# joeyan/gaussian_splatting

Hardware: AMD Instinct MI355X
Metric: forward+backward Mpixels/s @ ~1MP, N Gaussians; grad max-rel-err vs ref (higher is better)
Workload: dtype f32; 1 GPU; D: 2860000 Gaussians, 1297x840, SH degree 3, seed 0; N=2860000, V=2751015, P=1089480, camera=fixed, parallelism=single

## Files before the change

### gaussian_splatting_amd/csrc/gs_common.h

```cpp
#pragma once
#include <hip/hip_runtime.h>
#include <stdint.h>

#include "../../include/gsplat_hip.h"

#define GS_WAVE 64

namespace gs {

void set_error(const char* fmt, ...);
int check_launch(const char* what);

#define GS_REQUIRE(cond, ...)                                                                      \
    do {                                                                                           \
        if (!(cond)) {                                                                             \
            gs::set_error(__VA_ARGS__);                                                            \
            return GS_EINVAL;                                                                      \
        }                                                                                          \
    } while (0)

__host__ __device__ inline float bits_f(uint32_t u) {
    union { uint32_t u; float f; } c;
    c.u = u;
    return c.f;
// ... 24 lines not shown
    p = __builtin_fmaf(p, f, 1.33335581464284e-3f);
    p = __builtin_fmaf(p, f, 9.61812910762848e-3f);
    p = __builtin_fmaf(p, f, 5.55041086648216e-2f);
    p = __builtin_fmaf(p, f, 2.40226506959101e-1f);
    p = __builtin_fmaf(p, f, 6.93147180559945e-1f);
    p = __builtin_fmaf(p, f, 1.0f);
    float r = __builtin_ldexpf(p, (int)n);
    r = (t > 127.0f) ? __builtin_inff() : r;
    r = (t > -125.0f) ? r : 0.0f;
    r = (t != t) ? t : r;
    return r;
}

template <typename T> __device__ inline T gexp(T x);
template <> __device__ inline float gexp<float>(float x) { return det_expf(x); }
template <> __device__ inline double gexp<double>(double x) { return exp(x); }

template <typename T> __device__ inline T gsqrt(T x);
template <> __device__ inline float gsqrt<float>(float x) { return __builtin_sqrtf(x); }
template <> __device__ inline double gsqrt<double>(double x) { return __builtin_sqrt(x); }

__device__ inline int f2i(float x) {
    if (x != x) return 0;
    if (x >= 2147483648.0f) return 2147483647;
    if (x <= -2147483648.0f) return (-2147483647 - 1);
    return (int)x;
}

template <typename T, int RA, int CA, int CB>
__device__ inline void matmul(const T* A, const T* B, T* C) {
#pragma unroll
    for (int r = 0; r < RA; r++)
#pragma unroll
        for (int c = 0; c < CB; c++) {
            T sum = 0;
#pragma unroll
            for (int k = 0; k < CA; k++) sum += A[r * CA + k] * B[k * CB + c];
            C[r * CB + c] = sum;
        }
}
template <typename T, int R, int C>
__device__ inline void transp(const T* A, T* At) {
#pragma unroll
    for (int r = 0; r < R; r++)
#pragma unroll
        for (int c = 0; c < C; c++) At[c * R + r] = A[r * C + c];
}

#define GS_SH_0 0.28209479177387814f
#define GS_R_SH_0 3.544907701811032f
#define GS_SH_1 0.4886025119029199f
#define GS_SH_2_0 1.0925484305920792f
#define GS_SH_2_2 0.31539156525252005f
#define GS_SH_2_4 0.5462742152960396f
#define GS_SH_3_0 0.5900435899266435f
#define GS_SH_3_1 2.890611442640554f
#define GS_SH_3_2 0.4570457994644658f
#define GS_SH_3_3 0.263875515352797f
#define GS_SH_3_5 1.445305721320277f

template <typename T, int N_SH>
__device__ inline void sh_basis(const T* d, T* Y) {
    Y[0] = T(GS_SH_0);
    if constexpr (N_SH >= 4) {
        const T x = d[0], y = d[1], z = d[2];
        Y[1] = T(-GS_SH_1) * y;
        Y[2] = T(GS_SH_1) * z;
        Y[3] = T(-GS_SH_1) * x;
        if constexpr (N_SH >= 9) {
            const T xy = x * y, yz = y * z, xz = x * z, xx = x * x, yy = y * y, zz = z * z;
            Y[4] = T(GS_SH_2_0) * xy;
            Y[5] = T(-GS_SH_2_0) * yz;
            Y[6] = T(GS_SH_2_2) * (3 * zz - 1.0);
            Y[7] = T(-GS_SH_2_0) * xz;
            Y[8] = T(GS_SH_2_4) * (xx - yy);
            if constexpr (N_SH >= 16) {
                Y[9] = T(-GS_SH_3_0) * y * (3 * xx - yy);
                Y[10] = T(GS_SH_3_1) * xy * z;
                Y[11] = T(-GS_SH_3_2) * y * (5 * zz - 1.0);
                Y[12] = T(GS_SH_3_3) * z * (5 * zz - 3.0);
                Y[13] = T(-GS_SH_3_2) * x * (5 * zz - 1.0);
                Y[14] = T(GS_SH_3_5) * z * (xx - yy);
                Y[15] = T(-GS_SH_3_0) * x * (xx - 3 * yy);
            }
        }
    }
}

template <typename T, int N_SH>
__device__ inline void sh_to_rgb(const T* coeff, const T* Y, T* rgb) {
#pragma unroll
    for (int c = 0; c < 3; c++) rgb[c] = Y[0] * coeff[N_SH * c];
    if constexpr (N_SH >= 4) {
#pragma unroll
        for (int s = 1; s < N_SH; s++)
#pragma unroll
            for (int c = 0; c < 3; c++) rgb[c] += Y[s] * coeff[N_SH * c + s];
    }
}

template <typename T, int N_SH>
__device__ inline void sh_to_rgb_contracted(const T* coeff, const T* Y, T* rgb) {
#pragma clang fp contract(fast)
#pragma unroll
    for (int c = 0; c < 3; c++) rgb[c] = Y[0] * coeff[N_SH * c];
    if constexpr (N_SH >= 4) {
#pragma unroll
        for (int s = 1; s < N_SH; s++)
#pragma unroll
            for (int c = 0; c < 3; c++) rgb[c] += Y[s] * coeff[N_SH * c + s];
    }
}

constexpr int SORT_MAX_LDS_KEYS = 8192;
__host__ __device__ inline bool prefix_sorted_tile(int n, int sort_prefix) {
    return sort_prefix > 0 && n > sort_prefix && n <= SORT_MAX_LDS_KEYS;
}

int sort_flagged_tiles(const int* ranges, const uint64_t* keys, int* sorted, int tile0, int nt,
                       int64_t S, const int* flags, hipStream_t s);

constexpr int DC_PART = 256;
struct CutState {
    int* ctrl;
    int* totals;
    int* bstar;
    int* boff;
    int* boff2;
    uint32_t* bounds;
    int* phist;
    int* list;
    uint16_t* bucket_of;
};
__host__ __device__ inline size_t cut_ws_ints(int N, int T) {
    const size_t n = (size_t)(N > 0 ? N : 1), t = (size_t)(T > 0 ? T : 1);
    return 8 + 2 * t + 2 * (GS_CUT_BUCKETS + 8) + GS_CUT_BUCKETS + (size_t)DC_PART * GS_CUT_BUCKETS + n + (n + 1) / 2 + 16;
}
__host__ __device__ inline CutState cut_state_of(int32_t* ws, int N, int T) {
    const size_t n = (size_t)(N > 0 ? N : 1), t = (size_t)(T > 0 ? T : 1);
    CutState c;
    int* p = ws;
    c.ctrl = p; p += 8;
    c.totals = p; p += t;
    c.bstar = p; p += t;
    c.boff = p; p += GS_CUT_BUCKETS + 8;
    c.boff2 = p; p += GS_CUT_BUCKETS + 8;
    c.bounds = (uint32_t*)p; p += GS_CUT_BUCKETS;
    c.phist = p; p += (size_t)DC_PART * GS_CUT_BUCKETS;
    c.list = p; p += n;
    c.bucket_of = (uint16_t*)p;
    return c;
}

int depth_cut_repair(const float* bin_records, int N, int ntx, int nty, float mh, int row0, int row1,
                     const int* full_ranges, int32_t* workspace, int32_t* cut_ws, uint64_t* okeys, int64_t ocap,
                     int* osorted, const int* flags, hipStream_t s, bool sort_too = true);
int* depth_cut_flag_counter(int32_t* cut_ws, int N, int T);

inline int div_up(int a, int b) { return (a + b - 1) / b; }

}
```

### gaussian_splatting_amd/csrc/gs_error.hip

```cpp
#include <stdarg.h>
#include <stdio.h>

#include "gs_common.h"

namespace gs {

static thread_local char g_err[512] = "";

void set_error(const char* fmt, ...) {
    va_list ap;
    va_start(ap, fmt);
    vsnprintf(g_err, sizeof(g_err), fmt, ap);
    va_end(ap);
}

int check_launch(const char* what) {
    hipError_t e = hipGetLastError();
    if (e != hipSuccess) {
        set_error("%s: %s", what, hipGetErrorString(e));
        return GS_EHIP;
    }
    return GS_OK;
}

}

extern "C" {
const char* gs_last_error(void) { return gs::g_err; }
int gs_abi_version(void) { return 15; }
}
```

### gaussian_splatting_amd/csrc/preprocess.hip

```cpp
#include <type_traits>

#include "adam_math.h"
#include "pg_math.h"
#include "tile_math.h"

namespace gs {

constexpr int PP_BLOCK = 256;

struct Frustum {
    float near, far, u_lo, u_hi, v_lo, v_hi;
};

__device__ inline void camera_center(const float* __restrict__ M, float* __restrict__ center) {
    const double a = M[0], b = M[1], c = M[2], d = M[4], e = M[5], f = M[6], g = M[8], h = M[9],
                 i = M[10];
    const double tx = M[3], ty = M[7], tz = M[11];
    const double A = e * i - f * h, B = -(d * i - f * g), C = d * h - e * g;
    const double det = a * A + b * B + c * C;
    const double inv[9] = {A / det, -(b * i - c * h) / det, (b * f - c * e) / det,
                           B / det, (a * i - c * g) / det, -(a * f - c * d) / det,
                           C / det, -(a * h - b * g) / det, (a * e - b * d) / det};
    center[0] = (float)(-(inv[0] * tx + inv[1] * ty + inv[2] * tz));
    center[1] = (float)(-(inv[3] * tx + inv[4] * ty + inv[5] * tz));
    center[2] = (float)(-(inv[6] * tx + inv[7] * ty + inv[8] * tz));
}

__device__ inline void to_camera(const float* __restrict__ M, float x, float y, float z, float* c) {
    c[0] = M[0] * x + M[1] * y + M[2] * z + M[3];
    c[1] = M[4] * x + M[5] * y + M[6] * z + M[7];
    c[2] = M[8] * x + M[9] * y + M[10] * z + M[11];
}

__device__ inline bool is_culled(const float* c, const float* __restrict__ K, const Frustum& fr,
                                 float* uv) {
    uv[0] = K[0] * c[0] / c[2] + K[2];
    uv[1] = K[4] * c[1] / c[2] + K[5];
    return (c[2] < fr.near) | (c[2] > fr.far) | (uv[0] < fr.u_lo) | (uv[0] > fr.u_hi) |
           (uv[1] < fr.v_lo) | (uv[1] > fr.v_hi);
}

__device__ inline int depth_bin(float z, const Frustum& fr) {
    const uint32_t lo = sortable_bits(fr.near), hi = sortable_bits(fr.far);
    const uint64_t range = (uint64_t)(hi - lo) + 1;
    const uint32_t x = min(max(sortable_bits(z), lo), hi);
    return (int)(((uint64_t)(x - lo) * GS_CUT_HIST_BINS) / range);
}

__global__ __launch_bounds__(PP_BLOCK) void k_cull_count(const float* __restrict__ xyz,
                                                         const float* __restrict__ M,
                                                         const float* __restrict__ K, int N,
                                                         Frustum fr, int* __restrict__ block_counts,
                                                         float* __restrict__ center,
                                                         int* __restrict__ depth_hist, int sample_stride) {
    __shared__ int s_cnt[PP_BLOCK / GS_WAVE];
    const int g = blockIdx.x * PP_BLOCK + threadIdx.x;
    if (g == 0) camera_center(M, center);
    bool vis = false;
    if (g < N) {
        float c[3], uv[2];
        to_camera(M, xyz[g * 3 + 0], xyz[g * 3 + 1], xyz[g * 3 + 2], c);
        vis = !is_culled(c, K, fr, uv);
        if (depth_hist != nullptr && vis && g % sample_stride == 0)
            atomicAdd(&depth_hist[depth_bin(c[2], fr)], 1);
    }
    const int n = __popcll(__ballot(vis));
    if ((threadIdx.x & 63) == 0) s_cnt[threadIdx.x >> 6] = n;
    __syncthreads();
    if (threadIdx.x == 0) block_counts[blockIdx.x] = s_cnt[0] + s_cnt[1] + s_cnt[2] + s_cnt[3];
}

template <bool CUT>
__global__ __launch_bounds__(1024) void k_scan_counts(const int* __restrict__ counts, int n,
                                                      int* __restrict__ offsets,
                                                      int* __restrict__ total_out, int* __restrict__ depth_hist,
                                                      uint32_t* __restrict__ bounds, Frustum fr) {
    __shared__ int s_wave[16];
    __shared__ int s_carry;
    __shared__ int s_cum[CUT ? GS_CUT_HIST_BINS : 1];
    const int tid = threadIdx.x, lane = tid & 63, wave = tid >> 6;
    if constexpr (CUT) if (blockIdx.x == 1) {
        constexpr int PER = GS_CUT_HIST_BINS / 1024;
        static_assert(GS_CUT_HIST_BINS % 1024 == 0 && GS_CUT_BUCKETS == 1024, "one thread per bucket, PER bins per thread");
        int v[PER], sum = 0;
#pragma unroll
        for (int k = 0; k < PER; k++) {
            v[k] = depth_hist[tid * PER + k];
            depth_hist[tid * PER + k] = 0;
            sum += v[k];
        }
        int incl = sum;
#pragma unroll
        for (int d = 1; d < 64; d <<= 1) {
            const int o = __shfl_up(incl, d);
            if (lane >= d) incl += o;
        }
        if (lane == 63) s_wave[wave] = incl;
        __syncthreads();
        int run = incl - sum, valid = 0;
        for (int w = 0; w < 16; w++) {
            if (w < wave) run += s_wave[w];
            valid += s_wave[w];
        }
#pragma unroll
        for (int k = 0; k < PER; k++) {
            run += v[k];
            s_cum[tid * PER + k] = run;
        }
        __syncthreads();
        uint32_t bound = 0xffffffffu;
        if (tid < GS_CUT_BUCKETS - 1 && valid > 0) {
            const int64_t target_num = (int64_t)(tid + 1) * valid;
            int lo_i = 0, len = GS_CUT_HIST_BINS;
            while (len > 0) {
                const int half = len >> 1;
                if ((int64_t)s_cum[lo_i + half] * GS_CUT_BUCKETS < target_num) {
                    lo_i += half + 1;
                    len -= half + 1;
                } else {
                    len = half;
                }
            }
            const int j = min(lo_i, GS_CUT_HIST_BINS - 1);
            const int64_t prev = j > 0 ? s_cum[j - 1] : 0, h = max(s_cum[j] - (int)prev, 1);
            const uint32_t lo = sortable_bits(fr.near), hi = sortable_bits(fr.far);
            const uint64_t range = (uint64_t)(hi - lo) + 1;
            const double frac = (double)(target_num - prev * GS_CUT_BUCKETS) / ((double)h * GS_CUT_BUCKETS);
            const double pos = ((double)j + frac) / (double)GS_CUT_HIST_BINS;
            const uint64_t b = (uint64_t)lo + (uint64_t)(pos * (double)range);
            bound = (uint32_t)min(b, (uint64_t)hi);
        }
        if (tid < GS_CUT_BUCKETS) bounds[tid] = bound;
        return;
    }
    if (tid == 0) s_carry = 0;
    __syncthreads();
    for (int base = 0; base < n; base += 4096) {
        int v[4], sum = 0;
#pragma unroll
        for (int k = 0; k < 4; k++) {
            const int i = base + tid * 4 + k;
            v[k] = i < n ? counts[i] : 0;
            sum += v[k];
        }
        int incl = sum;
#pragma unroll
        for (int d = 1; d < 64; d <<= 1) {
            const int o = __shfl_up(incl, d);
            if (lane >= d) incl += o;
        }
        if (lane == 63) s_wave[wave] = incl;
        __syncthreads();
        int off = s_carry;
        for (int w = 0; w < wave; w++) off += s_wave[w];
        int run = off + incl - sum;
#pragma unroll
        for (int k = 0; k < 4; k++) {
            const int i = base + tid * 4 + k;
            if (i < n) offsets[i] = run;
            run += v[k];
        }
        __syncthreads();
        if (tid == 1023) s_carry = run;
        __syncthreads();
    }
    if (tid == 0) total_out[0] = s_carry;
}

__device__ inline float sigmoid_det(float x) { return 1.0f / (1.0f + det_expf(-x)); }

struct PreOut {
    float* uv;
    float* conic;
    float* opacity;
    float* rgb;
    float* xyz_cam;
    float* packed;
    int* vis_idx;
    int* rank;
    uint8_t* culled;
    float* bin_rec;
    const uint32_t* bounds;
    uint16_t* bucket_of;
};

struct Band {
    int row0, row1, ntx, nty;
    float mh;
};

template <int N_SH, bool BAND, bool AA = false>
__global__ __launch_bounds__(PP_BLOCK) __attribute__((amdgpu_waves_per_eu(5, 8))) void k_preprocess(
    const float* __restrict__ xyz, const float* __restrict__ quat, const float* __restrict__ scale,
    const float* __restrict__ opacity, const float* __restrict__ rgb, const float* __restrict__ sh,
    const float* __restrict__ M, const float* __restrict__ K, const float* __restrict__ center,
    int N, Frustum fr, const int* __restrict__ block_offsets, PreOut o, Band band) {
    __shared__ int s_cnt[PP_BLOCK / GS_WAVE];
    constexpr int SHW = 3 * (N_SH - 1);
    constexpr int HALF = PP_BLOCK / 2;
    __shared__ alignas(16) float s_sh[(N_SH > 1 && !BAND) ? HALF * SHW : 4];
    __shared__ uint32_t s_bounds[BAND ? 1 : GS_CUT_BUCKETS];
    const int g = blockIdx.x * PP_BLOCK + threadIdx.x;
    const int lane = threadIdx.x & 63, wave = threadIdx.x >> 6;
    if constexpr (!BAND) {
        if (o.bin_rec != nullptr)
            for (int k = threadIdx.x; k < GS_CUT_BUCKETS; k += PP_BLOCK) s_bounds[k] = o.bounds[k];
    }
    bool vis = false;
    float c[3] = {0, 0, 1}, uv[2] = {0, 0}, p[3] = {0, 0, 0};
    typedef float vfloat4 __attribute__((ext_vector_type(4)));
    constexpr int SH_PRE = (N_SH > 1 && !BAND) ? (HALF * SHW / 4 + PP_BLOCK - 1) / PP_BLOCK : 1;
    vfloat4 pre[2][SH_PRE];
    float q4[4] = {0, 0, 0, 1}, s3[3] = {0, 0, 0}, opa_raw = 0;
    if (g < N) {
        p[0] = xyz[g * 3 + 0]; p[1] = xyz[g * 3 + 1]; p[2] = xyz[g * 3 + 2];
        if constexpr (!BAND) {
            q4[0] = quat[g * 4 + 0]; q4[1] = quat[g * 4 + 1]; q4[2] = quat[g * 4 + 2]; q4[3] = quat[g * 4 + 3];
            s3[0] = scale[g * 3 + 0]; s3[1] = scale[g * 3 + 1]; s3[2] = scale[g * 3 + 2];
            opa_raw = opacity[g];
        }
    }
    if constexpr (N_SH > 1 && !BAND) {
// ... 754 lines not shown
#pragma unroll
        for (int k = 0; k < 3; k++) {
            adam_update(as_p[k], gs[k], as_m[k], as_v[k], S.w1, S.beta2, S.w2, ad.scale.bc2_sqrt, S.eps, ad.scale.neg_step);
            ad.scale.p[g * 3 + k] = as_p[k]; ad.scale.m[g * 3 + k] = as_m[k]; ad.scale.v[g * 3 + k] = as_v[k];
            adam_update(ac_p[k], gc[k], ac_m[k], ac_v[k], S.w1, S.beta2, S.w2, ad.rgb.bc2_sqrt, S.eps, ad.rgb.neg_step);
            ad.rgb.p[g * 3 + k] = ac_p[k]; ad.rgb.m[g * 3 + k] = ac_m[k]; ad.rgb.v[g * 3 + k] = ac_v[k];
        }
        adam_update(ao_p, go, ao_m, ao_v, S.w1, S.beta2, S.w2, ad.opacity.bc2_sqrt, S.eps, ad.opacity.neg_step);
        ad.opacity.p[g] = ao_p; ad.opacity.m[g] = ao_m; ad.opacity.v[g] = ao_v;
        return;
    }
    o.quaternion[g * 4 + 0] = gq[0]; o.quaternion[g * 4 + 1] = gq[1];
    o.quaternion[g * 4 + 2] = gq[2]; o.quaternion[g * 4 + 3] = gq[3];
    o.scale[g * 3 + 0] = gs[0]; o.scale[g * 3 + 1] = gs[1]; o.scale[g * 3 + 2] = gs[2];
    o.opacity[g] = go;
    o.rgb[g * 3 + 0] = gc[0]; o.rgb[g * 3 + 1] = gc[1]; o.rgb[g * 3 + 2] = gc[2];
}

constexpr int POSE_MAX_BLOCKS = 2048;
constexpr int POSE_SUM_BLOCK = 1024;

inline int pose_blocks(int N) {
    const int nb = N > 0 ? div_up(N, PP_BLOCK) : 0;
    return nb < POSE_MAX_BLOCKS ? nb : POSE_MAX_BLOCKS;
}

struct NoOpacity {};
template <bool AA = false>
__global__ __launch_bounds__(PP_BLOCK) void k_pose_bwd(
    const float* __restrict__ xyz, const float* __restrict__ quat, const float* __restrict__ scale,
    const float* __restrict__ M, const float* __restrict__ K, const int* __restrict__ rank,
    const float* __restrict__ g_slab, int v_base, int N, float* __restrict__ rows,
    std::conditional_t<AA, const float*, NoOpacity> opacity_act = {}) {
    __shared__ float s_part[PP_BLOCK / GS_WAVE][12];
    float acc[12];
#pragma unroll
    for (int k = 0; k < 12; k++) acc[k] = 0.0f;
    float W[9];
    load_rotation(M, W);
    const float fx = K[0], fy = K[4];
    for (int g = blockIdx.x * PP_BLOCK + threadIdx.x; g < N; g += gridDim.x * PP_BLOCK) {
        const int v = rank[g];
        if (v < 0) continue;
        const float* gsl = g_slab + (size_t)(v - v_base) * 9;
        const float p[3] = {xyz[g * 3 + 0], xyz[g * 3 + 1], xyz[g * 3 + 2]};
        const float q4[4] = {quat[g * 4 + 0], quat[g * 4 + 1], quat[g * 4 + 2], quat[g * 4 + 3]};
        const float s3[3] = {scale[g * 3 + 0], scale[g * 3 + 1], scale[g * 3 + 2]};
        float c[3], S9[9], J6[6], gJ6[6], gW9[9], gcam[3];
        to_camera(M, p[0], p[1], p[2], c);
        sigma_world_of(q4, s3, S9);
        const float z = c[2], z2 = c[2] * c[2];
        J6[0] = fx / z; J6[1] = 0; J6[2] = -fx * c[0] / z2;
        J6[3] = 0; J6[4] = fy / z; J6[5] = -fy * c[1] / z2;
        float gc3[3] = {gsl[6], gsl[7], gsl[8]};
        if constexpr (AA) {
            float c3[3], g_opa = gsl[3];
            conic_of(J6, W, S9, c3);
            aa_fold_row(aa_terms_of(c3), opacity_act[v], g_opa, gc3);
        }
        conic_bwd_pose_of(J6, W, S9, gc3, gJ6, gW9);
        cam_grad_of(c, fx, fy, gJ6, gsl + 4, gcam);
#pragma unroll
        for (int i = 0; i < 3; i++) {
#pragma unroll
            for (int j = 0; j < 3; j++) acc[4 * i + j] += gW9[3 * i + j] + gcam[i] * p[j];
            acc[4 * i + 3] += gcam[i];
        }
    }
#pragma unroll
    for (int k = 0; k < 12; k++)
#pragma unroll
        for (int d = 1; d < GS_WAVE; d <<= 1) acc[k] += __shfl_xor(acc[k], d);
    if ((threadIdx.x & (GS_WAVE - 1)) == 0)
#pragma unroll
        for (int k = 0; k < 12; k++) s_part[threadIdx.x / GS_WAVE][k] = acc[k];
    __syncthreads();
    static_assert(PP_BLOCK / GS_WAVE == 4, "the workgroup sum below names its four waves");
    if (threadIdx.x < 12)
        rows[blockIdx.x * 12 + threadIdx.x] = (s_part[0][threadIdx.x] + s_part[1][threadIdx.x]) +
                                              (s_part[2][threadIdx.x] + s_part[3][threadIdx.x]);
}

__global__ __launch_bounds__(POSE_SUM_BLOCK) void k_pose_sum(const float* __restrict__ rows, int n_rows,
                                                             float* __restrict__ out) {
    __shared__ double s_sum[POSE_SUM_BLOCK / 16][12];
    const int k = threadIdx.x & 15, r0 = threadIdx.x >> 4;
    if (k < 12) {
        double sum = 0.0;
        for (int r = r0; r < n_rows; r += POSE_SUM_BLOCK / 16) sum += (double)rows[(size_t)r * 12 + k];
        s_sum[r0][k] = sum;
    }
    __syncthreads();
    if (threadIdx.x < 12) {
        double sum = 0.0;
        for (int r = 0; r < POSE_SUM_BLOCK / 16; r++) sum += s_sum[r][threadIdx.x];
        out[threadIdx.x] = (float)sum;
    } else if (threadIdx.x < 16) {
        out[threadIdx.x] = 0.0f;
    }
}

}

using namespace gs;

static Frustum make_frustum(int W, int H, float near, float far, float padding) {
    Frustum fr;
    fr.near = near;
    fr.far = far;
    fr.u_lo = -1.0f * padding;
    fr.u_hi = (float)W + padding;
    fr.v_lo = -1.0f * padding;
    fr.v_hi = (float)H + padding;
    return fr;
}

#define DISPATCH_SH(n_sh, CALL)                                                                    \
    switch (n_sh) {                                                                                \
        case 1: { constexpr int N_SH = 1; CALL; } break;                                           \
        case 4: { constexpr int N_SH = 4; CALL; } break;                                           \
        case 9: { constexpr int N_SH = 9; CALL; } break;                                           \
        case 16: { constexpr int N_SH = 16; CALL; } break;                                         \
        default:                                                                                   \
            gs::set_error("Unsupported number of SH coefficients: %d", n_sh);                      \
            return GS_EINVAL;                                                                      \
    }

#define GS_RASTER_MODE(raster_mode, aa)                                                                      \
    GS_REQUIRE((raster_mode) == GS_RASTER_CLASSIC || (raster_mode) == GS_RASTER_ANTIALIASED,               \
               "raster_mode must be GS_RASTER_CLASSIC or GS_RASTER_ANTIALIASED, got %d", (int)(raster_mode)); \
    const bool aa = (raster_mode) == GS_RASTER_ANTIALIASED

static int preprocess_forward_launch(const void* xyz, const void* quaternion, const void* scale,
                                     const void* opacity, const void* rgb, const void* sh, int n_sh,
                                     const void* camera_T_world, const void* K, int N, int W, int H,
                                     float near_thresh, float far_thresh, float cull_mask_padding,
                                     float mh_dist, int band_row0, int band_row1,
                                     int32_t* workspace, void* camera_center, int32_t* visible_count,
                                     uint8_t* culling_mask, int32_t* rank, int32_t* vis_idx, void* uv,
                                     void* xyz_camera_frame, void* conic, void* opacity_act, void* rgb_render,
                                     void* packed, void* bin_records, int32_t* cut_workspace, int32_t* depth_hist,
                                     int sample_stride, bool aa, void* stream) {
    GS_REQUIRE((bin_records == nullptr) == (cut_workspace == nullptr) && (bin_records == nullptr) == (depth_hist == nullptr),
               "bin_records, cut_workspace and depth_hist go together");
    GS_REQUIRE(depth_hist == nullptr || sample_stride >= 1, "sample_stride must be gs_cut_sample_stride(N)");
    GS_REQUIRE(bin_records != nullptr || (uv != nullptr && xyz_camera_frame != nullptr && conic != nullptr),
               "uv, xyz_camera_frame and conic may only be omitted together with bin_records");
    GS_REQUIRE(n_sh == 1 || sh != nullptr, "sh must be given when n_sh > 1");
    hipStream_t s = (hipStream_t)stream;
    const Frustum fr = make_frustum(W, H, near_thresh, far_thresh, cull_mask_padding);
    const int nb = div_up(N > 0 ? N : 1, PP_BLOCK);
    int* block_counts = workspace;
    int* block_offsets = workspace + nb;
    k_cull_count<<<nb, PP_BLOCK, 0, s>>>((const float*)xyz, (const float*)camera_T_world,
                                         (const float*)K, N, fr, block_counts, (float*)camera_center, depth_hist,
                                         sample_stride > 0 ? sample_stride : 1);
    const int n_tiles = ((W + GS_TILE - 1) / GS_TILE) * ((H + GS_TILE - 1) / GS_TILE);
    CutState cs{};
    if (cut_workspace != nullptr) {
        cs = cut_state_of(cut_workspace, N, n_tiles);
        k_scan_counts<true><<<2, 1024, 0, s>>>(block_counts, nb, block_offsets, visible_count, depth_hist, cs.bounds, fr);
    } else {
        k_scan_counts<false><<<1, 1024, 0, s>>>(block_counts, nb, block_offsets, visible_count, nullptr, nullptr, fr);
    }
    PreOut o;
    o.uv = (float*)uv;
    o.conic = (float*)conic;
    o.opacity = (float*)opacity_act;
    o.rgb = (float*)rgb_render;
    o.xyz_cam = (float*)xyz_camera_frame;
    o.packed = (float*)packed;
    o.vis_idx = vis_idx;
    o.rank = rank;
    o.culled = culling_mask;
    o.bin_rec = (float*)bin_records;
    o.bounds = cs.bounds;
    o.bucket_of = cs.bucket_of;
    Band band;
    band.ntx = (W + GS_TILE - 1) / GS_TILE;
    band.nty = (H + GS_TILE - 1) / GS_TILE;
    band.row0 = band_row0;
    band.row1 = band_row1;
    band.mh = mh_dist;
    GS_REQUIRE(band_row0 >= 0 && band_row1 <= band.nty && band_row0 <= band_row1, "bad tile row band");
    const bool banded = !(band_row0 == 0 && band_row1 == band.nty);
    GS_REQUIRE(!(banded && bin_records != nullptr), "the depth-bucketed binning serves whole frames");
    GS_REQUIRE(!(banded && aa), "GS_RASTER_ANTIALIASED serves whole frames (no tile-row band)");
    if (aa) {
        DISPATCH_SH(n_sh, (k_preprocess<N_SH, false, true><<<nb, PP_BLOCK, 0, s>>>(
                              (const float*)xyz, (const float*)quaternion, (const float*)scale,
                              (const float*)opacity, (const float*)rgb, (const float*)sh,
                              (const float*)camera_T_world, (const float*)K,
                              (const float*)camera_center, N, fr, block_offsets, o, band)));
    } else if (banded) {
        DISPATCH_SH(n_sh, (k_preprocess<N_SH, true><<<nb, PP_BLOCK, 0, s>>>(
                              (const float*)xyz, (const float*)quaternion, (const float*)scale,
                              (const float*)opacity, (const float*)rgb, (const float*)sh,
                              (const float*)camera_T_world, (const float*)K,
                              (const float*)camera_center, N, fr, block_offsets, o, band)));
    } else {
        DISPATCH_SH(n_sh, (k_preprocess<N_SH, false><<<nb, PP_BLOCK, 0, s>>>(
                              (const float*)xyz, (const float*)quaternion, (const float*)scale,
                              (const float*)opacity, (const float*)rgb, (const float*)sh,
                              (const float*)camera_T_world, (const float*)K,
                              (const float*)camera_center, N, fr, block_offsets, o, band)));
    }
    return check_launch("preprocess_forward");
}

extern "C" {

size_t gs_preprocess_workspace_ints(int N) { return (size_t)div_up(N > 0 ? N : 1, PP_BLOCK) * 2 + 8; }

int gs_preprocess_forward_cut(const void* xyz, const void* quaternion, const void* scale,
                              const void* opacity, const void* rgb, const void* sh, int n_sh,
                              const void* camera_T_world, const void* K, int N, int W, int H,
                              float near_thresh, float far_thresh, float cull_mask_padding,
                              float mh_dist, int band_row0, int band_row1,
                              int32_t* workspace, void* camera_center, int32_t* visible_count,
                              uint8_t* culling_mask, int32_t* rank, int32_t* vis_idx, void* uv,
                              void* xyz_camera_frame, void* conic, void* opacity_act, void* rgb_render,
                              void* packed, void* bin_records, int32_t* cut_workspace, int32_t* depth_hist,
                              int sample_stride, void* stream) {
    return preprocess_forward_launch(xyz, quaternion, scale, opacity, rgb, sh, n_sh, camera_T_world, K, N, W, H, near_thresh,
                                     far_thresh, cull_mask_padding, mh_dist, band_row0, band_row1, workspace, camera_center,
                                     visible_count, culling_mask, rank, vis_idx, uv, xyz_camera_frame, conic, opacity_act,
                                     rgb_render, packed, bin_records, cut_workspace, depth_hist, sample_stride, false, stream);
}

int gs_preprocess_forward_mode(const void* xyz, const void* quaternion, const void* scale,
                               const void* opacity, const void* rgb, const void* sh, int n_sh,
                               const void* camera_T_world, const void* K, int N, int W, int H,
                               float near_thresh, float far_thresh, float cull_mask_padding,
                               float mh_dist, int band_row0, int band_row1,
                               int32_t* workspace, void* camera_center, int32_t* visible_count,
                               uint8_t* culling_mask, int32_t* rank, int32_t* vis_idx, void* uv,
                               void* xyz_camera_frame, void* conic, void* opacity_act, void* rgb_render,
                               void* packed, void* bin_records, int32_t* cut_workspace, int32_t* depth_hist,
                               int sample_stride, int raster_mode, void* stream) {
    GS_RASTER_MODE(raster_mode, aa);
    return preprocess_forward_launch(xyz, quaternion, scale, opacity, rgb, sh, n_sh, camera_T_world, K, N, W, H, near_thresh,
                                     far_thresh, cull_mask_padding, mh_dist, band_row0, band_row1, workspace, camera_center,
                                     visible_count, culling_mask, rank, vis_idx, uv, xyz_camera_frame, conic, opacity_act,
                                     rgb_render, packed, bin_records, cut_workspace, depth_hist, sample_stride, aa, stream);
}


int gs_band_project(const void* xyz, const void* scale, const void* opacity, const void* camera_T_world, const void* K,
                    int N, int W, int H, float near_thresh, float far_thresh, float cull_mask_padding, float mh_dist,
                    const int32_t* band_rows, int G, int32_t* workspace, void* camera_center, int32_t* visible_count,
                    uint8_t* culling_mask, int32_t* rank, int32_t* vis_idx, void* uv, void* opacity_act, uint32_t* mask,
                    int32_t* halo_workspace, void* stream) {
    GS_REQUIRE(G >= 1 && G <= GS_MAX_RANKS, "band_project: 1 <= G <= %d", GS_MAX_RANKS);
    hipStream_t s = (hipStream_t)stream;
    const Frustum fr = make_frustum(W, H, near_thresh, far_thresh, cull_mask_padding);
    const int nb = div_up(N > 0 ? N : 1, PP_BLOCK);
    int* block_counts = workspace;
    int* block_offsets = workspace + nb;
    k_cull_count<<<nb, PP_BLOCK, 0, s>>>((const float*)xyz, (const float*)camera_T_world, (const float*)K, N, fr,
                                         block_counts, (float*)camera_center, nullptr, 1);
    k_scan_counts<false><<<1, 1024, 0, s>>>(block_counts, nb, block_offsets, visible_count, nullptr, nullptr, fr);
    BandRows rows;
    for (int i = 0; i <= GS_MAX_RANKS; i++) rows.v[i] = i <= G ? band_rows[i] : 0;
    const int nty = (H + GS_TILE - 1) / GS_TILE;
    k_band_project<1><<<nb, PP_BLOCK, 0, s>>>((const float*)xyz, (const float*)scale, (const float*)opacity,
                                              (const float*)camera_T_world, (const float*)K, N, fr, mh_dist, nty, rows, G,
                                              block_offsets, culling_mask, rank, vis_idx, (float*)uv, (float*)opacity_act,
                                              mask, nullptr, nb);
    k_band_bit_counts<<<nb, PP_BLOCK, 0, s>>>(mask, visible_count, G, halo_workspace, nb);
    return check_launch("band_project");
}

int gs_preprocess_forward(const void* xyz, const void* quaternion, const void* scale,
                          const void* opacity, const void* rgb, const void* sh, int n_sh,
                          const void* camera_T_world, const void* K, int N, int W, int H,
                          float near_thresh, float far_thresh, float cull_mask_padding,
                          float mh_dist, int band_row0, int band_row1,
                          int32_t* workspace, void* camera_center, int32_t* visible_count,
                          uint8_t* culling_mask, int32_t* rank, int32_t* vis_idx, void* uv,
                          void* xyz_camera_frame, void* conic, void* opacity_act, void* rgb_render,
                          void* packed, void* stream) {
    return gs_preprocess_forward_cut(xyz, quaternion, scale, opacity, rgb, sh, n_sh, camera_T_world, K, N, W, H, near_thresh,
                                     far_thresh, cull_mask_padding, mh_dist, band_row0, band_row1, workspace, camera_center,
                                     visible_count, culling_mask, rank, vis_idx, uv, xyz_camera_frame, conic, opacity_act,
                                     rgb_render, packed, nullptr, nullptr, nullptr, 0, stream);
}

int gs_preprocess_forward_list(const void* xyz, const void* quaternion, const void* scale, const void* rgb, const void* sh,
                               int n_sh, const void* camera_T_world, const void* K, const void* camera_center,
                               const int32_t* list, const int32_t* list_count, int capacity, const int32_t* vis_idx,
                               const void* uv, const void* opacity_act, void* uv_l, void* xyz_camera_frame_l, void* conic_l,
                               void* packed_l, void* stream) {
    GS_REQUIRE(n_sh == 1 || sh != nullptr, "sh must be given when n_sh > 1");
    if (capacity <= 0) return GS_OK;
    hipStream_t s = (hipStream_t)stream;
    DISPATCH_SH(n_sh, (k_preprocess_list<N_SH><<<div_up(capacity, PP_BLOCK), PP_BLOCK, 0, s>>>(
                          (const float*)xyz, (const float*)quaternion, (const float*)scale, (const float*)rgb,
                          (const float*)sh, (const float*)camera_T_world, (const float*)K, (const float*)camera_center, list,
                          list_count, vis_idx, (const float*)uv, (const float*)opacity_act, (float*)uv_l,
                          (float*)xyz_camera_frame_l, (float*)conic_l, (float*)packed_l)));
    return check_launch("preprocess_forward_list");
}

namespace {
struct FrontendWs {
    int nb, nbp;
    int32_t *counts, *offsets;
    uint16_t* gmask;
};
FrontendWs frontend_ws(int32_t* workspace, int N, int G) {
    FrontendWs w;
    w.nb = div_up(N > 0 ? N : 1, PP_BLOCK);
    w.nbp = w.nb + 1;
    w.counts = workspace;
    w.offsets = workspace + (size_t)(G + 1) * w.nbp;
    w.gmask = reinterpret_cast<uint16_t*>(workspace + 2 * (size_t)(G + 1) * w.nbp);
    return w;
}
GatherPlan gather_plan(const FrontendWs& w, int G, int rank, const int32_t* owner_blocks, const void* recv,
                       const int32_t* recv_offsets) {
    GatherPlan gp;
    gp.gmask = w.gmask;
    gp.offsets = w.offsets;
    gp.recv = (const float*)recv;
    gp.nbp = w.nbp;
    gp.G = G;
    gp.blk0 = owner_blocks[rank] < w.nb ? owner_blocks[rank] : w.nb;
    for (int i = 0; i < GS_MAX_RANKS; i++) gp.recv_off[i] = i < G ? recv_offsets[i] : 0;
    return gp;
}
}

size_t gs_band_frontend_workspace_ints(int N, int G) {
    const size_t nbp = (size_t)div_up(N > 0 ? N : 1, PP_BLOCK) + 1;
    return 2 * (size_t)(G + 1) * nbp + ((size_t)(N > 0 ? N : 1) + 1) / 2;
}

int gs_band_frontend(const void* xyz, const void* quaternion, const void* scale, const void* opacity, const void* rgb,
                     const void* sh, int n_sh, const void* camera_T_world, const void* K, int N, int W, int H,
                     float near_thresh, float far_thresh, float cull_mask_padding, float mh_dist, const int32_t* band_rows,
                     const int32_t* owner_blocks, int G, int rank, int32_t* workspace, void* camera_center,
                     uint8_t* culling_mask, int32_t* rank_out, void* uv, void* opacity_act, int32_t* send_index,
                     int32_t* list_g, void* uv_l, void* xyz_camera_frame_l, void* conic_l, void* packed_l, int32_t* plan,
                     int32_t* plan_host, void* stream) {
    GS_REQUIRE(G >= 1 && G <= GS_MAX_RANKS, "band_frontend: 1 <= G <= %d", GS_MAX_RANKS);
    GS_REQUIRE(rank >= 0 && rank < G, "band_frontend: bad rank");
    GS_REQUIRE(N > 0, "band_frontend: N must be positive");
    GS_REQUIRE(n_sh == 1 || sh != nullptr, "sh must be given when n_sh > 1");
    hipStream_t s = (hipStream_t)stream;
    const Frustum fr = make_frustum(W, H, near_thresh, far_thresh, cull_mask_padding);
    const FrontendWs w = frontend_ws(workspace, N, G);
    BandRows rows;
    BandOwners owners;
    for (int i = 0; i <= GS_MAX_RANKS; i++) {
        rows.v[i] = i <= G ? band_rows[i] : 0;
        owners.v[i] = i <= G ? owner_blocks[i] : 0;
        GS_REQUIRE(i == 0 || i > G || owner_blocks[i] >= owner_blocks[i - 1], "band_frontend: owner_blocks must ascend");
    }
    const int nty = (H + GS_TILE - 1) / GS_TILE;
    k_band_count<<<w.nb, PP_BLOCK, 0, s>>>((const float*)xyz, (const float*)scale, (const float*)camera_T_world,
                                           (const float*)K, N, fr, mh_dist, nty, rows, G, w.counts, w.nbp, w.gmask,
                                           (float*)camera_center);
    k_band_scan<<<G + 1, 1024, 0, s>>>(w.counts, w.nb, w.nbp, w.offsets);
    k_band_write<<<w.nb + 1, PP_BLOCK, 0, s>>>((const float*)xyz, (const float*)opacity, (const float*)camera_T_world,
                                               (const float*)K, N, fr, w.gmask, w.offsets, w.nb, w.nbp, G, rank, owners,
                                               culling_mask, rank_out, (float*)uv, (float*)opacity_act, send_index, list_g,
                                               (float*)uv_l, (float*)xyz_camera_frame_l, (float*)conic_l, (float*)packed_l,
                                               plan, plan_host);
    const int32_t* list_count = w.offsets + (size_t)(1 + rank) * w.nbp + w.nb;
    DISPATCH_SH(n_sh, (k_band_rows<N_SH><<<w.nb, PP_BLOCK, 0, s>>>(
                          (const float*)quaternion, (const float*)scale, (const float*)rgb, (const float*)sh,
                          (const float*)camera_T_world, (const float*)K, (const float*)camera_center, list_g, list_count,
                          (const float*)uv_l, (const float*)xyz_camera_frame_l, (float*)conic_l, (float*)packed_l)));
    return check_launch("band_frontend");
}

int gs_band_gather_sum(const int32_t* workspace, int N, int G, int rank, const int32_t* owner_blocks,
                       const int32_t* rank_of_gaussian, int v_lo, const void* recv, const int32_t* recv_offsets, void* out,
                       void* stream) {
    GS_REQUIRE(G >= 1 && G <= GS_MAX_RANKS && rank >= 0 && rank < G, "band_gather_sum: bad G / rank");
    const FrontendWs w = frontend_ws(const_cast<int32_t*>(workspace), N, G);
    const GatherPlan gp = gather_plan(w, G, rank, owner_blocks, recv, recv_offsets);
    const int blk1 = owner_blocks[rank + 1] < w.nb ? owner_blocks[rank + 1] : w.nb;
    if (blk1 <= gp.blk0) return GS_OK;
    k_band_gather_sum<<<blk1 - gp.blk0, PP_BLOCK, 0, (hipStream_t)stream>>>(gp, N, rank_of_gaussian, v_lo, (float*)out);
    return check_launch("band_gather_sum");
}

int gs_preprocess_backward_gathered(const void* xyz, const void* quaternion, const void* scale, int n_sh,
                                    const void* camera_T_world, const void* K, const void* camera_center,
                                    const int32_t* rank_of_gaussian, const void* opacity_act, const int32_t* workspace,
                                    int N_total, int G, int rank, const int32_t* owner_blocks, const void* recv,
                                    const int32_t* recv_offsets, int n, void* grad_xyz, void* grad_quaternion,
                                    void* grad_scale, void* grad_opacity_logit, void* grad_rgb_param, void* grad_sh,
                                    void* stream) {
    GS_REQUIRE(n_sh == 1 || grad_sh != nullptr, "grad_sh must be given when n_sh > 1");
    GS_REQUIRE(G >= 1 && G <= GS_MAX_RANKS && rank >= 0 && rank < G, "preprocess_backward_gathered: bad G / rank");
    if (n <= 0) return GS_OK;
    const FrontendWs w = frontend_ws(const_cast<int32_t*>(workspace), N_total, G);
    const GatherPlan gp = gather_plan(w, G, rank, owner_blocks, recv, recv_offsets);
    GS_REQUIRE((size_t)gp.blk0 * PP_BLOCK + (size_t)n <= (size_t)N_total, "preprocess_backward_gathered: slice beyond N");
    PreGrad o;
    o.xyz = (float*)grad_xyz;
    o.quaternion = (float*)grad_quaternion;
    o.scale = (float*)grad_scale;
    o.opacity = (float*)grad_opacity_logit;
    o.rgb = (float*)grad_rgb_param;
    o.sh = (float*)grad_sh;
    DISPATCH_SH(n_sh, (k_preprocess_bwd<N_SH, true><<<div_up(n, PP_BLOCK), PP_BLOCK, 0, (hipStream_t)stream>>>(
                          (const float*)xyz, (const float*)quaternion, (const float*)scale, (const float*)camera_T_world,
                          (const float*)K, (const float*)camera_center, rank_of_gaussian, (const float*)opacity_act, nullptr,
                          0, n, o, gp)));
    return check_launch("preprocess_backward_gathered");
// ... 129 lines not shown
```

Measured before the change: 861.9 Mpixels/s.

## Build depth histogram in LDS per workgroup and reduce rows in a second kernel

```diff
diff --git a/gaussian_splatting_amd/csrc/gs_common.h b/gaussian_splatting_amd/csrc/gs_common.h
--- a/gaussian_splatting_amd/csrc/gs_common.h
+++ b/gaussian_splatting_amd/csrc/gs_common.h
@@ -200,6 +200,16 @@
     return c;
 }
 
+constexpr int CH_MAX_ROWS = 256;
+inline int* cull_hist_rows_of(const CutState& c) { return (int*)(((uintptr_t)c.phist + 15) & ~(uintptr_t)15); }
+inline int cull_hist_rows(int N) {
+    const size_t n = (size_t)(N > 0 ? N : 1);
+    const size_t fit = ((size_t)DC_PART * GS_CUT_BUCKETS + n + (n + 1) / 2) / GS_CUT_HIST_BINS;
+    const size_t groups = (n + 1023) / 1024;
+    const size_t r = groups < fit ? groups : fit;
+    return (int)(r < CH_MAX_ROWS ? r : CH_MAX_ROWS);
+}
+
 int depth_cut_repair(const float* bin_records, int N, int ntx, int nty, float mh, int row0, int row1,
                      const int* full_ranges, int32_t* workspace, int32_t* cut_ws, uint64_t* okeys, int64_t ocap,
                      int* osorted, const int* flags, hipStream_t s, bool sort_too = true);
diff --git a/gaussian_splatting_amd/csrc/gs_error.hip b/gaussian_splatting_amd/csrc/gs_error.hip
--- a/gaussian_splatting_amd/csrc/gs_error.hip
+++ b/gaussian_splatting_amd/csrc/gs_error.hip
@@ -27,5 +27,5 @@
 
 extern "C" {
 const char* gs_last_error(void) { return gs::g_err; }
-int gs_abi_version(void) { return 15; }
+int gs_abi_version(void) { return 16; }
 }
diff --git a/gaussian_splatting_amd/csrc/preprocess.hip b/gaussian_splatting_amd/csrc/preprocess.hip
--- a/gaussian_splatting_amd/csrc/preprocess.hip
+++ b/gaussian_splatting_amd/csrc/preprocess.hip
@@ -40,19 +40,32 @@
            (uv[1] < fr.v_lo) | (uv[1] > fr.v_hi);
 }
 
-__device__ inline int depth_bin(float z, const Frustum& fr) {
-    const uint32_t lo = sortable_bits(fr.near), hi = sortable_bits(fr.far);
-    const uint64_t range = (uint64_t)(hi - lo) + 1;
-    const uint32_t x = min(max(sortable_bits(z), lo), hi);
-    return (int)(((uint64_t)(x - lo) * GS_CUT_HIST_BINS) / range);
+struct DepthBins {
+    uint32_t lo, hi;
+    int64_t range;
+    double inv;
+};
+__device__ inline DepthBins depth_bins_of(const Frustum& fr) {
+    DepthBins d;
+    d.lo = sortable_bits(fr.near);
+    d.hi = sortable_bits(fr.far);
+    d.range = (int64_t)(d.hi - d.lo) + 1;
+    d.inv = (double)GS_CUT_HIST_BINS / (double)d.range;
+    return d;
+}
+__device__ inline int depth_bin(float z, const DepthBins& d) {
+    const uint32_t a = min(max(sortable_bits(z), d.lo), d.hi) - d.lo;
+    int q = (int)((double)a * d.inv);
+    const int64_t r = (int64_t)((uint64_t)a * GS_CUT_HIST_BINS) - (int64_t)q * d.range;
+    q += (int)(r >= d.range) - (int)(r < 0);
+    return min(max(q, 0), GS_CUT_HIST_BINS - 1);
 }
 
 __global__ __launch_bounds__(PP_BLOCK) void k_cull_count(const float* __restrict__ xyz,
                                                          const float* __restrict__ M,
                                                          const float* __restrict__ K, int N,
                                                          Frustum fr, int* __restrict__ block_counts,
-                                                         float* __restrict__ center,
-                                                         int* __restrict__ depth_hist, int sample_stride) {
+                                                         float* __restrict__ center) {
     __shared__ int s_cnt[PP_BLOCK / GS_WAVE];
     const int g = blockIdx.x * PP_BLOCK + threadIdx.x;
     if (g == 0) camera_center(M, center);
@@ -61,13 +74,105 @@
         float c[3], uv[2];
         to_camera(M, xyz[g * 3 + 0], xyz[g * 3 + 1], xyz[g * 3 + 2], c);
         vis = !is_culled(c, K, fr, uv);
-        if (depth_hist != nullptr && vis && g % sample_stride == 0)
-            atomicAdd(&depth_hist[depth_bin(c[2], fr)], 1);
     }
     const int n = __popcll(__ballot(vis));
     if ((threadIdx.x & 63) == 0) s_cnt[threadIdx.x >> 6] = n;
     __syncthreads();
     if (threadIdx.x == 0) block_counts[blockIdx.x] = s_cnt[0] + s_cnt[1] + s_cnt[2] + s_cnt[3];
+}
+
+constexpr int CH_BLOCK = 1024, CH_SUB = CH_BLOCK / PP_BLOCK, CH_UNROLL = 4, CH_TRIP = CH_SUB * CH_UNROLL;
+static_assert(GS_CUT_HIST_BINS % (4 * CH_BLOCK) == 0, "16-byte row stores, the same number per thread");
+struct CullTrip {
+    float p[CH_UNROLL][3];
+    bool in[CH_UNROLL];
+};
+__global__ __launch_bounds__(CH_BLOCK) void k_cull_count_hist(const float* __restrict__ xyz,
+                                                              const float* __restrict__ M,
+                                                              const float* __restrict__ K, int N, int nb,
+                                                              Frustum fr, int* __restrict__ block_counts,
+                                                              float* __restrict__ center, int* __restrict__ rows) {
+    __shared__ alignas(16) int s_hist[GS_CUT_HIST_BINS];
+    __shared__ int s_cnt[CH_UNROLL][CH_BLOCK / GS_WAVE];
+    const int tid = threadIdx.x, sub = tid / PP_BLOCK, t = tid % PP_BLOCK;
+    const int b0 = (int)((int64_t)blockIdx.x * nb / gridDim.x), b1 = (int)((int64_t)(blockIdx.x + 1) * nb / gridDim.x);
+    auto request = [&](int base, CullTrip& c) {
+#pragma unroll
+        for (int u = 0; u < CH_UNROLL; u++) {
+            const int blk = base + u * CH_SUB + sub;
+            const int g = blk * PP_BLOCK + t;
+            c.in[u] = blk < b1 && g < N;
+            const int gl = c.in[u] ? g : N - 1;
+            c.p[u][0] = xyz[gl * 3 + 0]; c.p[u][1] = xyz[gl * 3 + 1]; c.p[u][2] = xyz[gl * 3 + 2];
+        }
+    };
+    const DepthBins bins = depth_bins_of(fr);
+    auto count = [&](int base, const CullTrip& c) {
+#pragma unroll
+        for (int u = 0; u < CH_UNROLL; u++) {
+            bool vis = false;
+            if (c.in[u]) {
+                float cam[3], uv[2];
+                to_camera(M, c.p[u][0], c.p[u][1], c.p[u][2], cam);
+                vis = !is_culled(cam, K, fr, uv);
+                if (vis) atomicAdd(&s_hist[depth_bin(cam[2], bins)], 1);
+            }
+            const int n = __popcll(__ballot(vis));
+            if ((tid & 63) == 0) s_cnt[u][tid >> 6] = n;
+        }
+        __syncthreads();
+        if (tid < CH_TRIP) {
+            const int blk = base + tid;
+            const int* w = &s_cnt[tid / CH_SUB][(tid % CH_SUB) * (PP_BLOCK / GS_WAVE)];
+            if (blk < b1) block_counts[blk] = w[0] + w[1] + w[2] + w[3];
+        }
+        __syncthreads();
+    };
+    CullTrip even, odd;
+    request(b0, even);
+    for (int k = tid; k < GS_CUT_HIST_BINS; k += CH_BLOCK) s_hist[k] = 0;
+    if (blockIdx.x == 0 && tid == 0) camera_center(M, center);
+    __syncthreads();
+    for (int base = b0; base < b1; base += 2 * CH_TRIP) {
+        request(base + CH_TRIP, odd);
+        count(base, even);
+        if (base + CH_TRIP >= b1) break;
+        request(base + 2 * CH_TRIP, even);
+        count(base + CH_TRIP, odd);
+    }
+    typedef int vint4 __attribute__((ext_vector_type(4)));
+    vint4* row = reinterpret_cast<vint4*>(rows + (size_t)blockIdx.x * GS_CUT_HIST_BINS);
+    const vint4* src = reinterpret_cast<const vint4*>(s_hist);
+#pragma unroll
+    for (int k = 0; k < GS_CUT_HIST_BINS / (4 * CH_BLOCK); k++) row[k * CH_BLOCK + tid] = src[k * CH_BLOCK + tid];
+}
+
+constexpr int HR_BINS = 64, HR_SEGS = 1024 / (HR_BINS / 4);
+static_assert(GS_CUT_HIST_BINS % HR_BINS == 0 && CH_MAX_ROWS % HR_SEGS == 0, "whole workgroups, whole row strides");
+__global__ __launch_bounds__(1024) void k_depth_hist_reduce(const int* __restrict__ rows, int n_rows,
+                                                            int* __restrict__ depth_hist) {
+    typedef int vint4 __attribute__((ext_vector_type(4)));
+    __shared__ vint4 s_seg[HR_SEGS][HR_BINS / 4];
+    const int lt = threadIdx.x % (HR_BINS / 4), seg = threadIdx.x / (HR_BINS / 4);
+    const int bin = blockIdx.x * HR_BINS;
+    vint4 v[CH_MAX_ROWS / HR_SEGS];
+#pragma unroll
+    for (int k = 0; k < CH_MAX_ROWS / HR_SEGS; k++) {
+        const int r = k * HR_SEGS + seg;
+        v[k] = r < n_rows ? reinterpret_cast<const vint4*>(rows + (size_t)r * GS_CUT_HIST_BINS + bin)[lt] : vint4{0, 0, 0, 0};
+    }
+    vint4 sum = v[0];
+#pragma unroll
+    for (int k = 1; k < CH_MAX_ROWS / HR_SEGS; k++) sum += v[k];
+    s_seg[seg][lt] = sum;
+    __syncthreads();
+    if (threadIdx.x < HR_BINS) {
+        const int* col = reinterpret_cast<const int*>(&s_seg[0][0]) + threadIdx.x;
+        int total = 0;
+#pragma unroll 16
+        for (int s2 = 0; s2 < HR_SEGS; s2++) total += col[s2 * HR_BINS];
+        depth_hist[bin + threadIdx.x] = total;
+    }
 }
 
 template <bool CUT>
@@ -1128,15 +1233,23 @@
     const int nb = div_up(N > 0 ? N : 1, PP_BLOCK);
     int* block_counts = workspace;
     int* block_offsets = workspace + nb;
-    k_cull_count<<<nb, PP_BLOCK, 0, s>>>((const float*)xyz, (const float*)camera_T_world,
-                                         (const float*)K, N, fr, block_counts, (float*)camera_center, depth_hist,
-                                         sample_stride > 0 ? sample_stride : 1);
     const int n_tiles = ((W + GS_TILE - 1) / GS_TILE) * ((H + GS_TILE - 1) / GS_TILE);
     CutState cs{};
     if (cut_workspace != nullptr) {
         cs = cut_state_of(cut_workspace, N, n_tiles);
+        const int n_rows = N > 0 ? cull_hist_rows(N) : 0;
+        int* rows = cull_hist_rows_of(cs);
+        if (n_rows > 0)
+            k_cull_count_hist<<<n_rows, CH_BLOCK, 0, s>>>((const float*)xyz, (const float*)camera_T_world, (const float*)K, N,
+                                                          nb, fr, block_counts, (float*)camera_center, rows);
+        else
+            k_cull_count<<<nb, PP_BLOCK, 0, s>>>((const float*)xyz, (const float*)camera_T_world, (const float*)K, N, fr,
+                                                 block_counts, (float*)camera_center);
+        k_depth_hist_reduce<<<GS_CUT_HIST_BINS / HR_BINS, 1024, 0, s>>>(rows, n_rows, depth_hist);
         k_scan_counts<true><<<2, 1024, 0, s>>>(block_counts, nb, block_offsets, visible_count, depth_hist, cs.bounds, fr);
     } else {
+        k_cull_count<<<nb, PP_BLOCK, 0, s>>>((const float*)xyz, (const float*)camera_T_world,
+                                             (const float*)K, N, fr, block_counts, (float*)camera_center);
         k_scan_counts<false><<<1, 1024, 0, s>>>(block_counts, nb, block_offsets, visible_count, nullptr, nullptr, fr);
     }
     PreOut o;
@@ -1234,7 +1347,7 @@
     int* block_counts = workspace;
     int* block_offsets = workspace + nb;
     k_cull_count<<<nb, PP_BLOCK, 0, s>>>((const float*)xyz, (const float*)camera_T_world, (const float*)K, N, fr,
-                                         block_counts, (float*)camera_center, nullptr, 1);
+                                         block_counts, (float*)camera_center);
     k_scan_counts<false><<<1, 1024, 0, s>>>(block_counts, nb, block_offsets, visible_count, nullptr, nullptr, fr);
     BandRows rows;
     for (int i = 0; i <= GS_MAX_RANKS; i++) rows.v[i] = i <= G ? band_rows[i] : 0;
```

Result: faster. 871.9 Mpixels/s (median of 6 runs) (+1.2%).
